# HuiGuanLab/Lite-MKD

Measured on AMD Instinct MI355X. Metric: episodes/sec (5-way 5-shot, 8x224^2 frames), higher is better.
Workload: dtype f32

## Files before the change

### lite-mkd_amd/csrc/norm_pool.hip

```cpp
#include "common.h"
#include <vector>
#include <cmath>
#include <algorithm>

#define NP_THREADS 256
static int g_ew_wg_per_cu = 4;
extern "C" int lmkd_set_elementwise_wg_per_cu(int n) {
  LMKD_REQUIRE(n >= 1 && n <= 8, "lmkd_set_elementwise_wg_per_cu: %d outside 1..8 (the BatchNorm partial buffers hold 2048 rows)", n);
  g_ew_wg_per_cu = n;
  return LMKD_OK;
}
static inline int ew_grid(long n_items) {
  long g = (n_items + NP_THREADS - 1) / NP_THREADS;
  if (g > 256 * g_ew_wg_per_cu) g = 256 * g_ew_wg_per_cu;
  if (g < 1) g = 1;
  return (int)g;
}

extern "C" long lmkd_amax_words(void) { return 2 * LMKD_AMAX_SEG_WORDS; }
static inline unsigned* amd_out(const lmkd_amax_desc* d) { return d ? (unsigned*)d->out_words : nullptr; }
static inline const unsigned* amd_ref(const lmkd_amax_desc* d) { return (d && d->out_words) ? (const unsigned*)d->ref_words : nullptr; }

#define LMKD_FENCE_MAX 128
struct FenceArgs { const unsigned* w[LMKD_FENCE_MAX]; unsigned* r[LMKD_FENCE_MAX]; };
// ... 425 lines not shown
  LMKD_REQUIRE(partial && stats && scratch && tickets && T > 0 && C > 0 && count > 0, "lmkd_bn_finalize: bad arguments");
  LMKD_REQUIRE(cdiv(2 * C, CS_COLS) <= LMKD_TICKET_WORDS, "lmkd_bn_finalize: C=%d exceeds the ticket buffer", C);
  hipLaunchKernelGGL(bn_finalize_kernel, dim3(cdiv(2 * C, CS_COLS), cs_slices(T)), dim3(CS_COLS, CS_LANES), 0, (hipStream_t)stream, partial, T,
                     C, (double)count, gamma, beta, running_mean, running_var, momentum, eps, stats, scratch, tickets, 0, 0.0, 0, 0, bin, bout,
                     bout && amd ? (const unsigned*)amd->ref_words : nullptr);
  LMKD_CHECK_LAUNCH("bn_finalize_kernel");
  return LMKD_OK;
}

extern "C" int lmkd_bn_finalize_seg(const float* partial, int T, int T0, int C, long count0, long count1, const float* gamma, const float* beta,
                                    float eps, float* stats, double* scratch, unsigned* tickets, void* stream, const lmkd_amax_desc* amd) {
  const unsigned* bin = amd ? (const unsigned*)amd->x_words : nullptr;
  unsigned* bout = amd ? (unsigned*)amd->out_words : nullptr;
  if (!bin || !bout) { bin = nullptr; bout = nullptr; }
  LMKD_REQUIRE(partial && stats && scratch && tickets && T0 > 0 && T > T0 && C > 0 && count0 > 0 && count1 > 0, "lmkd_bn_finalize_seg: bad arguments");
  LMKD_REQUIRE(cdiv(2 * C, CS_COLS) <= LMKD_TICKET_WORDS / 2, "lmkd_bn_finalize_seg: C=%d exceeds the ticket buffer", C);
  const int S0 = cs_slices(T0), S1 = cs_slices(T - T0);
  hipLaunchKernelGGL(bn_finalize_kernel, dim3(cdiv(2 * C, CS_COLS), std::max(S0, S1), 2), dim3(CS_COLS, CS_LANES), 0, (hipStream_t)stream, partial, T,
                     C, (double)count0, gamma, beta, (float*)nullptr, (float*)nullptr, 0.f, eps, stats, scratch, tickets, T0, (double)count1, S0, S1, bin, bout,
                     bout && amd ? (const unsigned*)amd->ref_words : nullptr);
  LMKD_CHECK_LAUNCH("bn_finalize_kernel");
  return LMKD_OK;
}

extern "C" int lmkd_bn_eval_stats(int C, const float* gamma, const float* beta, const float* running_mean,
                                  const float* running_var, float eps, float* stats, void* stream) {
  LMKD_REQUIRE(running_mean && running_var && stats && C > 0, "lmkd_bn_eval_stats: bad arguments");
  hipLaunchKernelGGL(bn_eval_stats_kernel, dim3(cdiv(C, 64)), dim3(64), 0, (hipStream_t)stream, C, gamma, beta, running_mean,
                     running_var, eps, stats);
  LMKD_CHECK_LAUNCH("bn_eval_stats_kernel");
  return LMKD_OK;
}

template <typename T>
__global__ void bn_apply_kernel(const T* __restrict__ x, const float* __restrict__ stats, const T* __restrict__ res,
                                const float* __restrict__ rstats, T* __restrict__ y, long n4, int C, int relu, int res_mode,
                                unsigned* __restrict__ mask_bits, long n4_0, unsigned* __restrict__ amax, const unsigned* __restrict__ aref) {
  constexpr int U = ActU<T>::U;
  const int C4 = C >> 2;
  const long nu = n4 / U;
  AmaxStat am = {0.f, 0.f, 0u}, am1 = {0.f, 0.f, 0u};
  const AmaxRef rf0 = amax_ref(aref ? amax_read(aref, 0) : 0u), rf1 = amax_ref(aref ? amax_read(aref, 1) : 0u);
  for (long iu = (long)blockIdx.x * blockDim.x + threadIdx.x; iu < nu; iu += (long)gridDim.x * blockDim.x) {
    float4 v[U], r[U];
    ldv<T, U>(x, iu, v);
    if (res_mode) ldv<T, U>(res, iu, r);
    unsigned nibs = 0;
    const int so = iu * U >= n4_0 ? 5 * C : 0;
#pragma unroll
    for (int u = 0; u < U; ++u) {
      const long i = iu * U + u;
      const int c = (int)(i % C4) * 4 + so;
      const float4 sc = *reinterpret_cast<const float4*>(stats + 2 * C + c);
      const float4 sh = *reinterpret_cast<const float4*>(stats + 3 * C + c);
      float4& w = v[u];
      w.x = fmaf(w.x, sc.x, sh.x); w.y = fmaf(w.y, sc.y, sh.y); w.z = fmaf(w.z, sc.z, sh.z); w.w = fmaf(w.w, sc.w, sh.w);
      if (res_mode == 1) {
        w.x += r[u].x; w.y += r[u].y; w.z += r[u].z; w.w += r[u].w;
      } else if (res_mode == 2) {
        const float4 rs = *reinterpret_cast<const float4*>(rstats + 2 * C + c);
        const float4 rh = *reinterpret_cast<const float4*>(rstats + 3 * C + c);
        w.x += fmaf(r[u].x, rs.x, rh.x); w.y += fmaf(r[u].y, rs.y, rh.y); w.z += fmaf(r[u].z, rs.z, rh.z); w.w += fmaf(r[u].w, rs.w, rh.w);
      }
      if (relu) { w.x = fmaxf(w.x, 0.f); w.y = fmaxf(w.y, 0.f); w.z = fmaxf(w.z, 0.f); w.w = fmaxf(w.w, 0.f); }
      nibs |= ((w.x > 0.f ? 1u : 0u) | (w.y > 0.f ? 2u : 0u) | (w.z > 0.f ? 4u : 0u) | (w.w > 0.f ? 8u : 0u)) << (4 * u);
      if (so) amax_stat4(am1, w, rf1); else amax_stat4(am, w, rf0);
    }
    stv<T, U>(y, iu, v);
    if (mask_bits) {
      constexpr int LPW = 8 / U;
      unsigned wbits = nibs << (4 * U * (threadIdx.x & (LPW - 1)));
      wbits |= __shfl_xor(wbits, 1, 64);
      wbits |= __shfl_xor(wbits, 2, 64);
      if (LPW == 8) wbits |= __shfl_xor(wbits, 4, 64);
      if ((threadIdx.x & (LPW - 1)) == 0) mask_bits[iu / LPW] = wbits;
    }
  }
  if (amax) {
    amax_commit_stat(amax, am, aref != nullptr);
    if (n4_0 < n4) amax_commit_stat(amax + LMKD_AMAX_SEG_WORDS, am1, aref != nullptr);
  }
}

extern "C" int lmkd_bn_apply_seg(const float* x, const float* stats, const float* res, const float* rstats, float* y, long rows, long rows0,
                                 int C, int relu, int res_mode, unsigned* mask_bits, void* stream, const lmkd_amax_desc* amd);
extern "C" int lmkd_bn_apply(const float* x, const float* stats, const float* res, const float* rstats, float* y, long rows,
                             int C, int relu, int res_mode, unsigned* mask_bits, void* stream) {
  return lmkd_bn_apply_seg(x, stats, res, rstats, y, rows, rows, C, relu, res_mode, mask_bits, stream, nullptr);
}
extern "C" int lmkd_bn_apply_seg(const float* x, const float* stats, const float* res, const float* rstats, float* y, long rows, long rows0,
                                 int C, int relu, int res_mode, unsigned* mask_bits, void* stream, const lmkd_amax_desc* amd) {
  unsigned* amax = amd_out(amd);
  const unsigned* aref = amd_ref(amd);
  LMKD_REQUIRE(x && stats && y && rows > 0 && C > 0 && C % 4 == 0, "lmkd_bn_apply: bad arguments (C=%d)", C);
  if (rows0 <= 0 || rows0 > rows) rows0 = rows;
  LMKD_REQUIRE(res_mode == 0 || res, "lmkd_bn_apply: residual pointer missing");
  LMKD_REQUIRE(res_mode != 2 || rstats, "lmkd_bn_apply: residual stats missing");
  LMKD_REQUIRE(!mask_bits || C % 32 == 0, "lmkd_bn_apply: the ReLU bit mask needs C %% 32 == 0 (C=%d)", C);
  LMKD_REQUIRE(!g_lmkd_act_bf16 || C % 8 == 0, "lmkd_bn_apply: bf16 tensors need C %% 8 == 0 (C=%d)", C);
  const long n4 = rows * C / 4;
  if (g_lmkd_act_bf16)
    hipLaunchKernelGGL(bn_apply_kernel<lmkd_bf16_t>, dim3(ew_grid(n4)), dim3(NP_THREADS), 0, (hipStream_t)stream, (const lmkd_bf16_t*)x, stats,
                       (const lmkd_bf16_t*)res, rstats, (lmkd_bf16_t*)y, n4, C, relu, res_mode, mask_bits, rows0 * C / 4, amax, aref);
  else
    hipLaunchKernelGGL(bn_apply_kernel<float>, dim3(ew_grid(n4)), dim3(NP_THREADS), 0, (hipStream_t)stream, x, stats, res, rstats, y, n4, C,
                       relu, res_mode, mask_bits, rows0 * C / 4, amax, aref);
  LMKD_CHECK_LAUNCH("bn_apply_kernel");
  return LMKD_OK;
}

template <typename T>
__device__ __forceinline__ float4 bn_masked_grad(const float4 dy, const float4 xv, const T* yact, long i, const float* stats,
                                                 int C, int c, int mask_mode) {
  float4 g = dy;
  if (mask_mode == 3) {
    const unsigned nib = (reinterpret_cast<const unsigned*>(yact)[i >> 3] >> (4 * (int)(i & 7))) & 15u;
    g.x = (nib & 1u) ? g.x : 0.f; g.y = (nib & 2u) ? g.y : 0.f; g.z = (nib & 4u) ? g.z : 0.f; g.w = (nib & 8u) ? g.w : 0.f;
  } else if (mask_mode == 1) {
    const float4 yv = ld4<T>(yact, i);
    g.x = yv.x > 0.f ? g.x : 0.f; g.y = yv.y > 0.f ? g.y : 0.f; g.z = yv.z > 0.f ? g.z : 0.f; g.w = yv.w > 0.f ? g.w : 0.f;
  } else if (mask_mode == 2) {
    const float4 sc = *reinterpret_cast<const float4*>(stats + 2 * C + c);
    const float4 sh = *reinterpret_cast<const float4*>(stats + 3 * C + c);
    g.x = fmaf(xv.x, sc.x, sh.x) > 0.f ? g.x : 0.f; g.y = fmaf(xv.y, sc.y, sh.y) > 0.f ? g.y : 0.f;
    g.z = fmaf(xv.z, sc.z, sh.z) > 0.f ? g.z : 0.f; g.w = fmaf(xv.w, sc.w, sh.w) > 0.f ? g.w : 0.f;
  }
  return g;
}

struct BnSeg { long rows0; int nb1; };
template <typename T>
__global__ void bn_bwd_reduce_kernel(const T* __restrict__ dy, const T* __restrict__ x, const T* __restrict__ yact,
                                     const float* __restrict__ stats, float* __restrict__ partial, long rows, int C, int CC,
                                     int mask_mode, int nbv, BnSeg sg) {
  extern __shared__ float sm[];
  constexpr int U = ActU<T>::U;
  if (gridDim.z > 1) {
    if (blockIdx.z) {
      const long eo = sg.rows0 * C;
      dy += eo; x += eo;
      if (yact) yact = mask_mode == 3 ? reinterpret_cast<const T*>(reinterpret_cast<const unsigned*>(yact) + eo / 32) : yact + eo;
      stats += 5 * C; partial += (long)2048 * 2 * C; rows -= sg.rows0; nbv = sg.nb1;
    } else {
      rows = sg.rows0;
    }
  }
  const int C4 = C >> 2, CCV = CC / (4 * U);
  const int RL = NP_THREADS / CCV, RL1 = RL / U;
  const int cq = threadIdx.x % CCV, rl = threadIdx.x / CCV;
  const int bv = blockIdx.x * U + rl / RL1, vl = rl % RL1;
  const int c0 = blockIdx.y * CC;
  const int c = c0 + cq * 4 * U;
  float4 s1[U], s2[U], mean[U], istd[U];
#pragma unroll
  for (int u = 0; u < U; ++u) {
    s1[u] = make_float4(0, 0, 0, 0); s2[u] = make_float4(0, 0, 0, 0);
    mean[u] = *reinterpret_cast<const float4*>(stats + c + 4 * u);
    istd[u] = *reinterpret_cast<const float4*>(stats + C + c + 4 * u);
  }
  for (long r = bv < nbv ? (long)bv * RL1 + vl : rows; r < rows; r += (long)nbv * RL1) {
    const long i0 = r * C4 + (c >> 2);
    float4 xv[U], dv[U];
    ldv<T, U>(x, i0 / U, xv);
    ldv<T, U>(dy, i0 / U, dv);
#pragma unroll
    for (int u = 0; u < U; ++u) {
      const float4 g = bn_masked_grad<T>(dv[u], xv[u], yact, i0 + u, stats, C, c + 4 * u, mask_mode);
      s1[u].x += g.x; s1[u].y += g.y; s1[u].z += g.z; s1[u].w += g.w;
      s2[u].x = fmaf(g.x, (xv[u].x - mean[u].x) * istd[u].x, s2[u].x); s2[u].y = fmaf(g.y, (xv[u].y - mean[u].y) * istd[u].y, s2[u].y);
      s2[u].z = fmaf(g.z, (xv[u].z - mean[u].z) * istd[u].z, s2[u].z); s2[u].w = fmaf(g.w, (xv[u].w - mean[u].w) * istd[u].w, s2[u].w);
    }
  }
#pragma unroll
  for (int u = 0; u < U; ++u) {
    float* d = sm + ((long)rl * CC + cq * 4 * U + 4 * u) * 2;
    d[0] = s1[u].x; d[1] = s2[u].x; d[2] = s1[u].y; d[3] = s2[u].y; d[4] = s1[u].z; d[5] = s2[u].z; d[6] = s1[u].w; d[7] = s2[u].w;
  }
  __syncthreads();
  for (int j = threadIdx.x; j < 2 * CC; j += NP_THREADS) {
#pragma unroll
    for (int h = 0; h < U; ++h) {
      if (blockIdx.x * U + h >= nbv) break;
      float s = 0.f;
      for (int q = h * RL1; q < (h + 1) * RL1; ++q) s += sm[(long)q * 2 * CC + j];
      partial[(long)(blockIdx.x * U + h) * 2 * C + 2 * c0 + j] = s;
    }
  }
}

// ... 1 lines not shown
__global__ void bn_bwd_coef_kernel(const float* __restrict__ part, int T, int C, double count, const float* __restrict__ gamma,
                                   const float* __restrict__ stats, float* __restrict__ coef, float* __restrict__ dgamma,
                                   float* __restrict__ dbeta, int accumulate, double* __restrict__ scratch, unsigned* __restrict__ tickets,
                                   CoefSeg cs) {
  __shared__ double sm[CS_LANES][CS_COLS];
  __shared__ double tot[CS_COLS];
  __shared__ int s_last;
  int S = 0;
  const bool seg = gridDim.z > 1;
  if (seg) {
    if (blockIdx.z) { part += cs.pstride; T = cs.T1; count = cs.count1; stats += 5 * C; coef += 5 * C; scratch += (long)(CS_MAX_SLICES + 2) * 2 * C; tickets += LMKD_TICKET_WORDS / 2; S = cs.S1; }
    else S = cs.S0;
  }
  if (!colsum_ticket(part, T, 2 * C, scratch, tickets, sm, tot, &s_last, nullptr, S)) return;
  const int c = blockIdx.x * (CS_COLS / 2) + threadIdx.x;
  if (threadIdx.y != 0 || threadIdx.x >= CS_COLS / 2 || c >= C) return;
  const double sg = tot[2 * threadIdx.x], sgx = tot[2 * threadIdx.x + 1];
  const float g = gamma ? gamma[c] : 1.f;
  const float invstd = stats[C + c];
  coef[c] = g * invstd;
  coef[C + c] = (float)(sg / count);
  coef[2 * C + c] = (float)(sgx / count);
  if (seg) {
    coef[3 * C + c] = (float)sgx;
    coef[4 * C + c] = (float)sg;
    return;
  }
  if (dgamma) dgamma[c] = accumulate ? dgamma[c] + (float)sgx : (float)sgx;
  if (dbeta) dbeta[c] = accumulate ? dbeta[c] + (float)sg : (float)sg;
}

struct ParamGradSeg { float* dgamma; float* dbeta; int accumulate; };
__device__ __forceinline__ void bn_param_grads_seg(const float* __restrict__ coef, int C, const ParamGradSeg& pg) {
  if (blockIdx.x != 0 || !pg.dgamma) return;
  for (int c = threadIdx.x; c < C; c += blockDim.x) {
    const float gx = coef[3 * C + c] + coef[5 * C + 3 * C + c], g = coef[4 * C + c] + coef[5 * C + 4 * C + c];
    pg.dgamma[c] = pg.accumulate ? pg.dgamma[c] + gx : gx;
    if (pg.dbeta) pg.dbeta[c] = pg.accumulate ? pg.dbeta[c] + g : g;
  }
}

template <typename T>
__global__ void bn_bwd_apply_kernel(const T* __restrict__ dy, const T* __restrict__ x, const T* __restrict__ yact,
                                    const float* __restrict__ stats, const float* __restrict__ coef, T* __restrict__ dx,
                                    T* __restrict__ g_out, long n4, int C, int mask_mode, long n4_0, ParamGradSeg pg,
                                    unsigned* __restrict__ amax, const unsigned* __restrict__ aref) {
  constexpr int U = ActU<T>::U;
  const int C4 = C >> 2;
  const long nu = n4 / U;
  if (n4_0 < n4) bn_param_grads_seg(coef, C, pg);
  AmaxStat am = {0.f, 0.f, 0u}, am1 = {0.f, 0.f, 0u};
  const AmaxRef rf0 = amax_ref(aref ? amax_read(aref, 0) : 0u), rf1 = amax_ref(aref ? amax_read(aref, 1) : 0u);
  for (long iu = (long)blockIdx.x * blockDim.x + threadIdx.x; iu < nu; iu += (long)gridDim.x * blockDim.x) {
    float4 xv[U], dv[U], o[U], gq[U];
    ldv<T, U>(x, iu, xv);
    ldv<T, U>(dy, iu, dv);
    const int so = iu * U >= n4_0 ? 5 * C : 0;
    const float* st = stats + so;
    const float* cf = coef + so;
#pragma unroll
    for (int u = 0; u < U; ++u) {
      const long i = iu * U + u;
      const int c = (int)(i % C4) * 4;
      const float4 g = bn_masked_grad<T>(dv[u], xv[u], yact, i, st, C, c, mask_mode);
      const float4 mean = *reinterpret_cast<const float4*>(st + c);
      const float4 istd = *reinterpret_cast<const float4*>(st + C + c);
      const float4 A = *reinterpret_cast<const float4*>(cf + c);
      const float4 mg = *reinterpret_cast<const float4*>(cf + C + c);
      const float4 mgx = *reinterpret_cast<const float4*>(cf + 2 * C + c);
      o[u].x = A.x * (g.x - mg.x - (xv[u].x - mean.x) * istd.x * mgx.x);
      o[u].y = A.y * (g.y - mg.y - (xv[u].y - mean.y) * istd.y * mgx.y);
      o[u].z = A.z * (g.z - mg.z - (xv[u].z - mean.z) * istd.z * mgx.z);
      o[u].w = A.w * (g.w - mg.w - (xv[u].w - mean.w) * istd.w * mgx.w);
      gq[u] = g;
      if (so) amax_stat4(am1, o[u], rf1); else amax_stat4(am, o[u], rf0);
    }
    stv<T, U>(dx, iu, o);
    if (g_out) stv<T, U>(g_out, iu, gq);
  }
  if (amax) {
    amax_commit_stat(amax, am, aref != nullptr);
    if (n4_0 < n4) amax_commit_stat(amax + LMKD_AMAX_SEG_WORDS, am1, aref != nullptr);
  }
}

extern "C" long lmkd_bn_bwd_workspace(int C) { return (long)(2048 * 2 * C) * sizeof(float) + (long)(66 * 2 * C) * sizeof(double) + 64; }

static int bn_bwd_stats_impl(const float* dy, const float* x, const float* yact, const float* stats, const float* gamma, float* dgamma,
                             float* dbeta, float* coef, void* workspace, unsigned* tickets, long rows, long count, int C, int mask_mode,
                             int accumulate_param_grads, hipStream_t s, const char* who, long rows0 = 0, long count0 = 0) {
  LMKD_REQUIRE(dy && x && stats && coef && workspace && tickets, "%s: null pointer", who);
  const bool seg = rows0 > 0 && rows0 < rows;
  LMKD_REQUIRE(!seg || cdiv(2 * C, CS_COLS) <= LMKD_TICKET_WORDS / 2, "%s: C=%d exceeds the ticket buffer", who, C);
  const int CC = C > 1024 ? 1024 : C;
  const int U = g_lmkd_act_bf16 ? 2 : 1;
  LMKD_REQUIRE(C % (4 * U) == 0 && C % CC == 0 && 256 % (CC / 4) == 0, "%s: unsupported channel count %d", who, C);
  LMKD_REQUIRE((mask_mode != 1 && mask_mode != 3) || yact, "%s: mask_mode 1 / 3 needs the activation output / its bit mask", who);
  LMKD_REQUIRE(mask_mode != 3 || C % 32 == 0, "%s: bit masks need C %% 32 == 0", who);
  LMKD_REQUIRE(cdiv(2 * C, CS_COLS) <= LMKD_TICKET_WORDS, "%s: C=%d exceeds the ticket buffer", who, C);
  const int RL1 = NP_THREADS / (CC / 4), RL = RL1 * U;
  auto blocks = [&](long r) {
    int nb = cdiv(r, (long)RL1 * 8);
    if (nb > 256 * g_ew_wg_per_cu * 2) nb = 256 * g_ew_wg_per_cu * 2;
    if (nb > 2048) nb = 2048;
    return nb < 1 ? 1 : nb;
  };
  const int nb = blocks(seg ? rows0 : rows), nb1 = seg ? blocks(rows - rows0) : 0;
  const int nbx = std::max(nb, nb1);
  float* partial = (float*)workspace;
  double* dscr = (double*)((char*)workspace + (((long)(seg ? 2 : 1) * 2048 * 2 * C * sizeof(float) + 63) / 64) * 64);
  BnSeg bs;
  bs.rows0 = seg ? rows0 : rows; bs.nb1 = nb1;
  const int gz = seg ? 2 : 1;
  if (g_lmkd_act_bf16)
    hipLaunchKernelGGL(bn_bwd_reduce_kernel<lmkd_bf16_t>, dim3(cdiv(nbx, 2), C / CC, gz), dim3(NP_THREADS), (size_t)RL * CC * 2 * sizeof(float), s,
                       (const lmkd_bf16_t*)dy, (const lmkd_bf16_t*)x, (const lmkd_bf16_t*)yact, stats, partial, rows, C, CC, mask_mode, nb, bs);
  else
    hipLaunchKernelGGL(bn_bwd_reduce_kernel<float>, dim3(nbx, C / CC, gz), dim3(NP_THREADS), (size_t)RL * CC * 2 * sizeof(float), s, dy, x, yact,
                       stats, partial, rows, C, CC, mask_mode, nb, bs);
  LMKD_CHECK_LAUNCH("bn_bwd_reduce_kernel");
  CoefSeg cs;
  cs.T1 = nb1; cs.pstride = (long)2048 * 2 * C; cs.count1 = (double)(count - count0); cs.S0 = cs_slices(nb); cs.S1 = seg ? cs_slices(nb1) : 0;
  hipLaunchKernelGGL(bn_bwd_coef_kernel, dim3(cdiv(2 * C, CS_COLS), std::max(cs.S0, cs.S1), gz), dim3(CS_COLS, CS_LANES), 0, s, (const float*)partial, nb, C,
                     (double)(seg ? count0 : count), gamma, stats, coef, dgamma, dbeta, accumulate_param_grads, dscr, tickets, cs);
  LMKD_CHECK_LAUNCH("bn_bwd_coef_kernel");
  return LMKD_OK;
}

extern "C" int lmkd_bn_backward_seg(const float* dy, const float* x, const float* yact, const float* stats, const float* gamma, float* dx,
                                    float* g_out, float* dgamma, float* dbeta, float* coef, void* workspace, unsigned* tickets, long rows,
                                    long rows0, int C, int mask_mode, int accumulate_param_grads, void* stream, const lmkd_amax_desc* amd);
extern "C" int lmkd_bn_backward(const float* dy, const float* x, const float* yact, const float* stats, const float* gamma,
                                float* dx, float* g_out, float* dgamma, float* dbeta, float* coef, void* workspace, unsigned* tickets,
                                long rows, int C, int mask_mode, int accumulate_param_grads, void* stream) {
  return lmkd_bn_backward_seg(dy, x, yact, stats, gamma, dx, g_out, dgamma, dbeta, coef, workspace, tickets, rows, rows, C, mask_mode,
                              accumulate_param_grads, stream, nullptr);
}
extern "C" int lmkd_bn_backward_seg(const float* dy, const float* x, const float* yact, const float* stats, const float* gamma, float* dx,
                                    float* g_out, float* dgamma, float* dbeta, float* coef, void* workspace, unsigned* tickets, long rows,
                                    long rows0, int C, int mask_mode, int accumulate_param_grads, void* stream, const lmkd_amax_desc* amd) {
  unsigned* amax = amd_out(amd);
  const unsigned* aref = amd_ref(amd);
  LMKD_REQUIRE(dx, "lmkd_bn_backward: null pointer");
  hipStream_t s = (hipStream_t)stream;
  if (rows0 <= 0 || rows0 >= rows) rows0 = rows;
  const int rc = bn_bwd_stats_impl(dy, x, yact, stats, gamma, dgamma, dbeta, coef, workspace, tickets, rows, rows, C, mask_mode,
                                   accumulate_param_grads, s, "lmkd_bn_backward", rows0, rows0);
  if (rc) return rc;
  const long n4 = rows * C / 4, n4_0 = rows0 * C / 4;
  ParamGradSeg pg;
  pg.dgamma = dgamma; pg.dbeta = dbeta; pg.accumulate = accumulate_param_grads;
  if (g_lmkd_act_bf16)
    hipLaunchKernelGGL(bn_bwd_apply_kernel<lmkd_bf16_t>, dim3(ew_grid(n4)), dim3(NP_THREADS), 0, s, (const lmkd_bf16_t*)dy, (const lmkd_bf16_t*)x,
                       (const lmkd_bf16_t*)yact, stats, (const float*)coef, (lmkd_bf16_t*)dx, (lmkd_bf16_t*)g_out, n4, C, mask_mode, n4_0, pg, amax, aref);
  else
    hipLaunchKernelGGL(bn_bwd_apply_kernel<float>, dim3(ew_grid(n4)), dim3(NP_THREADS), 0, s, dy, x, yact, stats, (const float*)coef, dx, g_out,
                       n4, C, mask_mode, n4_0, pg, amax, aref);
  LMKD_CHECK_LAUNCH("bn_bwd_apply_kernel");
  return LMKD_OK;
}

extern "C" int lmkd_bn_backward_part_seg(const float* part, int T, int T0, const float* dy, const float* x, const float* stats, const float* gamma,
                                         float* dx, float* dgamma, float* dbeta, float* coef, void* workspace, unsigned* tickets, long rows,
                                         long rows0, int C, int accumulate_param_grads, void* stream, const lmkd_amax_desc* amd);
extern "C" int lmkd_bn_backward_part(const float* part, int T, const float* dy, const float* x, const float* stats, const float* gamma,
                                     float* dx, float* dgamma, float* dbeta, float* coef, void* workspace, unsigned* tickets, long rows, int C,
                                     int accumulate_param_grads, void* stream) {
  return lmkd_bn_backward_part_seg(part, T, T, dy, x, stats, gamma, dx, dgamma, dbeta, coef, workspace, tickets, rows, rows, C,
                                   accumulate_param_grads, stream, nullptr);
}
extern "C" int lmkd_bn_backward_part_seg(const float* part, int T, int T0, const float* dy, const float* x, const float* stats, const float* gamma,
                                         float* dx, float* dgamma, float* dbeta, float* coef, void* workspace, unsigned* tickets, long rows,
                                         long rows0, int C, int accumulate_param_grads, void* stream, const lmkd_amax_desc* amd) {
  unsigned* amax = amd_out(amd);
  const unsigned* aref = amd_ref(amd);
  LMKD_REQUIRE(part && T > 0 && dy && x && stats && dx && coef && workspace && tickets, "lmkd_bn_backward_part: null pointer");
  LMKD_REQUIRE(!g_lmkd_act_bf16 && C % 4 == 0, "lmkd_bn_backward_part: fp32 tensors, C %% 4 == 0");
  const bool seg = T0 > 0 && T0 < T && rows0 > 0 && rows0 < rows;
  LMKD_REQUIRE(seg || (T0 == T && rows0 == rows), "lmkd_bn_backward_part_seg: T0 / rows0 must both name a split or both the whole");
  LMKD_REQUIRE(cdiv(2 * C, CS_COLS) <= LMKD_TICKET_WORDS / (seg ? 2 : 1), "lmkd_bn_backward_part: C=%d exceeds the ticket buffer", C);
  hipStream_t s = (hipStream_t)stream;
  double* dscr = (double*)((char*)workspace + (((long)2048 * 2 * C * sizeof(float) + 63) / 64) * 64);
  CoefSeg cs;
  cs.T1 = T - T0; cs.pstride = (long)T0 * 2 * C; cs.count1 = (double)(rows - rows0); cs.S0 = cs_slices(T0); cs.S1 = seg ? cs_slices(T - T0) : 0;
  hipLaunchKernelGGL(bn_bwd_coef_kernel, dim3(cdiv(2 * C, CS_COLS), std::max(cs.S0, cs.S1), seg ? 2 : 1), dim3(CS_COLS, CS_LANES), 0, s, part, T0, C,
                     (double)rows0, gamma, stats, coef, dgamma, dbeta, accumulate_param_grads, dscr, tickets, cs);
  LMKD_CHECK_LAUNCH("bn_bwd_coef_kernel");
  const long n4 = rows * C / 4;
  ParamGradSeg pg;
  pg.dgamma = dgamma; pg.dbeta = dbeta; pg.accumulate = accumulate_param_grads;
  hipLaunchKernelGGL(bn_bwd_apply_kernel<float>, dim3(ew_grid(n4)), dim3(NP_THREADS), 0, s, dy, x, (const float*)nullptr, stats, (const float*)coef,
                     dx, (float*)nullptr, n4, C, 2, rows0 * C / 4, pg, amax, aref);
  LMKD_CHECK_LAUNCH("bn_bwd_apply_kernel");
  return LMKD_OK;
}

extern "C" int lmkd_bn_backward_stats(const float* dy, const float* cmax, const float* stats, const float* gamma, float* dgamma, float* dbeta,
                                      float* coef, void* workspace, unsigned* tickets, long pooled_rows, long count, int C,
                                      int accumulate_param_grads, void* stream) {
  LMKD_REQUIRE(pooled_rows > 0 && count >= pooled_rows, "lmkd_bn_backward_stats: bad row counts");
  return bn_bwd_stats_impl(dy, cmax, nullptr, stats, gamma, dgamma, dbeta, coef, workspace, tickets, pooled_rows, count, C, 2,
                           accumulate_param_grads, (hipStream_t)stream, "lmkd_bn_backward_stats");
}
extern "C" int lmkd_bn_backward_stats_seg(const float* dy, const float* cmax, const float* stats, const float* gamma, float* coef, void* workspace,
                                          unsigned* tickets, long pooled_rows, long pooled_rows0, long count, long count0, int C, void* stream) {
  LMKD_REQUIRE(pooled_rows0 > 0 && pooled_rows0 < pooled_rows && count0 >= pooled_rows0 && count - count0 >= pooled_rows - pooled_rows0,
               "lmkd_bn_backward_stats_seg: bad row counts");
  return bn_bwd_stats_impl(dy, cmax, nullptr, stats, gamma, nullptr, nullptr, coef, workspace, tickets, pooled_rows, count, C, 2, 0,
                           (hipStream_t)stream, "lmkd_bn_backward_stats_seg", pooled_rows0, count0);
}

template <typename T>
__global__ void relu_bwd_kernel(const T* __restrict__ dy, const T* __restrict__ y, T* __restrict__ g, long n4) {
  for (long i = (long)blockIdx.x * blockDim.x + threadIdx.x; i < n4; i += (long)gridDim.x * blockDim.x) {
    const float4 d = ld4<T>(dy, i), v = ld4<T>(y, i);
    st4<T>(g, i, make_float4(v.x > 0.f ? d.x : 0.f, v.y > 0.f ? d.y : 0.f, v.z > 0.f ? d.z : 0.f, v.w > 0.f ? d.w : 0.f));
  }
}
extern "C" int lmkd_relu_backward(const float* dy, const float* y, float* g, long n, void* stream) {
  LMKD_REQUIRE(dy && y && g && n > 0 && n % 4 == 0, "lmkd_relu_backward: bad arguments");
  if (g_lmkd_act_bf16)
    hipLaunchKernelGGL(relu_bwd_kernel<lmkd_bf16_t>, dim3(ew_grid(n / 4)), dim3(NP_THREADS), 0, (hipStream_t)stream, (const lmkd_bf16_t*)dy,
                       (const lmkd_bf16_t*)y, (lmkd_bf16_t*)g, n / 4);
  else
    hipLaunchKernelGGL(relu_bwd_kernel<float>, dim3(ew_grid(n / 4)), dim3(NP_THREADS), 0, (hipStream_t)stream, dy, y, g, n / 4);
  LMKD_CHECK_LAUNCH("relu_bwd_kernel");
  return LMKD_OK;
}

template <typename T>
__global__ void bn_relu_maxpool_kernel(const T* __restrict__ x, const float* __restrict__ stats, T* __restrict__ y,
                                       uchar4* __restrict__ idx, T* __restrict__ cmax, int N, int H, int W, int C, int OH, int OW, int N0,
                                       unsigned* __restrict__ amax, const unsigned* __restrict__ aref) {
  constexpr int U = ActU<T>::U;
  const int CU = C / (4 * U);
  const long total = (long)N * OH * OW * CU;
  AmaxStat amx = {0.f, 0.f, 0u}, amx1 = {0.f, 0.f, 0u};
  const AmaxRef rf0 = amax_ref(aref ? amax_read(aref, 0) : 0u), rf1 = amax_ref(aref ? amax_read(aref, 1) : 0u);
  for (long i = (long)blockIdx.x * blockDim.x + threadIdx.x; i < total; i += (long)gridDim.x * blockDim.x) {
    const int cq = (int)(i % CU);
    long r = i / CU;
    const int ow = (int)(r % OW); r /= OW;
    const int oh = (int)(r % OH);
    const int n = (int)(r / OH);
    float4 sc[U], sh[U], m[U], cm[U];
    uchar4 am[U];
#pragma unroll
    for (int u = 0; u < U; ++u) {
      const float* st = stats + (n >= N0 ? 5 * C : 0);
      sc[u] = *reinterpret_cast<const float4*>(st + 2 * C + (cq * U + u) * 4);
      sh[u] = *reinterpret_cast<const float4*>(st + 3 * C + (cq * U + u) * 4);
      m[u] = make_float4(-INFINITY, -INFINITY, -INFINITY, -INFINITY);
      cm[u] = make_float4(0.f, 0.f, 0.f, 0.f);
      am[u] = make_uchar4(255, 255, 255, 255);
    }
#pragma unroll
    for (int kh = 0; kh < 3; ++kh) {
      const int h = oh * 2 - 1 + kh;
      if ((unsigned)h >= (unsigned)H) continue;
#pragma unroll
      for (int kw = 0; kw < 3; ++kw) {
        const int w = ow * 2 - 1 + kw;
        if ((unsigned)w >= (unsigned)W) continue;
        float4 rr[U];
        ldv<T, U>(x, ((long)(n * H + h) * W + w) * CU + cq, rr);
        const unsigned char t = (unsigned char)(kh * 3 + kw);
#pragma unroll
        for (int u = 0; u < U; ++u) {
          const float4 r4 = rr[u];
          float4 v;
          v.x = fmaxf(fmaf(r4.x, sc[u].x, sh[u].x), 0.f); v.y = fmaxf(fmaf(r4.y, sc[u].y, sh[u].y), 0.f);
          v.z = fmaxf(fmaf(r4.z, sc[u].z, sh[u].z), 0.f); v.w = fmaxf(fmaf(r4.w, sc[u].w, sh[u].w), 0.f);
          if (v.x > m[u].x || am[u].x == 255) { m[u].x = v.x; am[u].x = t; cm[u].x = r4.x; }
          if (v.y > m[u].y || am[u].y == 255) { m[u].y = v.y; am[u].y = t; cm[u].y = r4.y; }
          if (v.z > m[u].z || am[u].z == 255) { m[u].z = v.z; am[u].z = t; cm[u].z = r4.z; }
          if (v.w > m[u].w || am[u].w == 255) { m[u].w = v.w; am[u].w = t; cm[u].w = r4.w; }
        }
      }
    }
    stv<T, U>(y, i, m);
#pragma unroll
    for (int u = 0; u < U; ++u) {
      idx[i * U + u] = am[u];
      if (n >= N0) amax_stat4(amx1, m[u], rf1); else amax_stat4(amx, m[u], rf0);
    }
    if (cmax) stv<T, U>(cmax, i, cm);
  }
  if (amax) {
    amax_commit_stat(amax, amx, aref != nullptr);
    if (N0 < N) amax_commit_stat(amax + LMKD_AMAX_SEG_WORDS, amx1, aref != nullptr);
  }
}

extern "C" int lmkd_bn_relu_maxpool_fwd_seg(const float* x, const float* stats, float* y, unsigned char* idx, float* cmax, int N, int N0, int H,
                                            int W, int C, void* stream, const lmkd_amax_desc* amd);
extern "C" int lmkd_bn_relu_maxpool_fwd(const float* x, const float* stats, float* y, unsigned char* idx, float* cmax, int N, int H, int W,
                                        int C, void* stream) {
  return lmkd_bn_relu_maxpool_fwd_seg(x, stats, y, idx, cmax, N, N, H, W, C, stream, nullptr);
}
extern "C" int lmkd_bn_relu_maxpool_fwd_seg(const float* x, const float* stats, float* y, unsigned char* idx, float* cmax, int N, int N0, int H,
                                            int W, int C, void* stream, const lmkd_amax_desc* amd) {
  unsigned* amax = amd_out(amd);
  const unsigned* aref = amd_ref(amd);
  LMKD_REQUIRE(x && stats && y && idx && C % (g_lmkd_act_bf16 ? 8 : 4) == 0, "lmkd_bn_relu_maxpool_fwd: bad arguments");
  if (N0 <= 0 || N0 > N) N0 = N;
  const int OH = (H + 2 - 3) / 2 + 1, OW = (W + 2 - 3) / 2 + 1;
  const long total = (long)N * OH * OW * C / (g_lmkd_act_bf16 ? 8 : 4);
  if (g_lmkd_act_bf16)
    hipLaunchKernelGGL(bn_relu_maxpool_kernel<lmkd_bf16_t>, dim3(ew_grid(total)), dim3(NP_THREADS), 0, (hipStream_t)stream, (const lmkd_bf16_t*)x,
                       stats, (lmkd_bf16_t*)y, (uchar4*)idx, (lmkd_bf16_t*)cmax, N, H, W, C, OH, OW, N0, amax, aref);
  else
    hipLaunchKernelGGL(bn_relu_maxpool_kernel<float>, dim3(ew_grid(total)), dim3(NP_THREADS), 0, (hipStream_t)stream, x, stats, y, (uchar4*)idx,
                       cmax, N, H, W, C, OH, OW, N0, amax, aref);
  LMKD_CHECK_LAUNCH("bn_relu_maxpool_kernel");
  return LMKD_OK;
}

template <typename T>
__global__ void maxpool_bwd_kernel(const T* __restrict__ dy, const uchar4* __restrict__ idx, T* __restrict__ g, int N, int H,
                                   int W, int C, int OH, int OW) {
  const int C4 = C >> 2;
  const long total = (long)N * H * W * C4;
  for (long i = (long)blockIdx.x * blockDim.x + threadIdx.x; i < total; i += (long)gridDim.x * blockDim.x) {
    const int cq = (int)(i % C4);
    long r = i / C4;
    const int w = (int)(r % W); r /= W;
    const int h = (int)(r % H);
    const int n = (int)(r / H);
    float4 acc = make_float4(0.f, 0.f, 0.f, 0.f);
    const int oh_lo = h >> 1, oh_hi = (h + 1) >> 1;
    const int ow_lo = w >> 1, ow_hi = (w + 1) >> 1;
    for (int oh = oh_lo; oh <= oh_hi; ++oh) {
      if (oh >= OH) continue;
      const int kh = h - (2 * oh - 1);
      for (int ow = ow_lo; ow <= ow_hi; ++ow) {
        if (ow >= OW) continue;
        const int kw = w - (2 * ow - 1);
        const unsigned char t = (unsigned char)(kh * 3 + kw);
        const long o = ((long)(n * OH + oh) * OW + ow) * C4 + cq;
        const uchar4 am = idx[o];
        const float4 d = ld4<T>(dy, o);
        if (am.x == t) acc.x += d.x;
        if (am.y == t) acc.y += d.y;
        if (am.z == t) acc.z += d.z;
        if (am.w == t) acc.w += d.w;
      }
    }
    st4<T>(g, i, acc);
  }
}

template <typename T>
__global__ void stem_unpool_bn_bwd_kernel(const T* __restrict__ dy, const uchar4* __restrict__ idx, const T* __restrict__ c,
                                          const float* __restrict__ stats, const float* __restrict__ coef, T* __restrict__ dc, int N,
                                          int H, int W, int C, int OH, int OW, int N0, ParamGradSeg pg, unsigned* __restrict__ amax,
                                          const unsigned* __restrict__ aref) {
  const int C4 = C >> 2;
  const int HB = (H + 1) >> 1, WB = (W + 1) >> 1;
  const long total = (long)N * HB * WB * C4;
  AmaxStat amx = {0.f, 0.f, 0u}, amx1 = {0.f, 0.f, 0u};
  const AmaxRef rf0 = amax_ref(aref ? amax_read(aref, 0) : 0u), rf1 = amax_ref(aref ? amax_read(aref, 1) : 0u);
  if (N0 < N) bn_param_grads_seg(coef, C, pg);
  for (long i = (long)blockIdx.x * blockDim.x + threadIdx.x; i < total; i += (long)gridDim.x * blockDim.x) {
    const int cq = (int)(i % C4);
    long r = i / C4;
    const int b = (int)(r % WB); r /= WB;
    const int a = (int)(r % HB);
    const int n = (int)(r / HB);
    const int ch = cq * 4 + (n >= N0 ? 5 * C : 0);
    const float4 sc = *reinterpret_cast<const float4*>(stats + 2 * C + ch);
    const float4 sh = *reinterpret_cast<const float4*>(stats + 3 * C + ch);
    const float4 mean = *reinterpret_cast<const float4*>(stats + ch);
    const float4 istd = *reinterpret_cast<const float4*>(stats + C + ch);
    const float4 A = *reinterpret_cast<const float4*>(coef + ch);
    const float4 mg = *reinterpret_cast<const float4*>(coef + C + ch);
    const float4 mgx = *reinterpret_cast<const float4*>(coef + 2 * C + ch);
    float4 d[2][2];
    uchar4 am[2][2];
#pragma unroll
    for (int wi = 0; wi < 2; ++wi)
#pragma unroll
      for (int wj = 0; wj < 2; ++wj) {
        const int oh = a + wi, ow = b + wj;
        if (oh < OH && ow < OW) {
          const long o = ((long)(n * OH + oh) * OW + ow) * C4 + cq;
          d[wi][wj] = ld4<T>(dy, o);
          am[wi][wj] = idx[o];
        } else {
          d[wi][wj] = make_float4(0.f, 0.f, 0.f, 0.f);
          am[wi][wj] = make_uchar4(254, 254, 254, 254);
        }
      }
#pragma unroll
    for (int pi = 0; pi < 2; ++pi) {
      const int h = 2 * a + pi;
      if (h >= H) continue;
// ... 186 lines not shown
```

Before: 51.01.

## Add specialized fp32 BatchNorm apply, backward-apply and BN-ReLU-maxpool kernels with LDS tables

Adds fp32-only kernels for BN apply, BN backward apply and fused BN+ReLU+maxpool. Each block processes one contiguous chunk, keeps the channel index with an incremental counter instead of a modulo, and uses 32-bit byte offsets. Per-channel scale/shift/coef values are staged in shared memory when C<=512. The aim is to cut integer division, 64-bit address arithmetic and redundant global loads of per-channel parameters in these bandwidth-bound passes, at the cost of extra code paths and 32-bit size limits.

```diff
diff --git a/lite-mkd_amd/csrc/norm_pool.hip b/lite-mkd_amd/csrc/norm_pool.hip
--- a/lite-mkd_amd/csrc/norm_pool.hip
+++ b/lite-mkd_amd/csrc/norm_pool.hip
@@ -531,6 +531,96 @@
   }
 }
 
+#define NP_TAB_MAX_C 512
+struct EwChunk { unsigned chunk, cmod; };
+static inline int ew_chunks(long n4, int C4, EwChunk* ck) {
+  const long g = ew_grid(n4);
+  const long chunk = ((n4 + g - 1) / g + NP_THREADS - 1) / NP_THREADS * NP_THREADS;
+  ck->chunk = (unsigned)chunk; ck->cmod = (unsigned)(chunk % C4);
+  return (int)((n4 + chunk - 1) / chunk);
+}
+#define LMKD_REQUIRE_EW32(n4, who) LMKD_REQUIRE((n4) < (1L << 31), "%s: %ld groups of 4 elements exceed the 32-bit offsets of the fp32 pass", who, (long)(n4))
+template <bool L>
+__device__ __forceinline__ float4 ew_row(const float4* __restrict__ s, const float* __restrict__ g, int row, int C4, unsigned c4) {
+  if constexpr (L) return s[row * C4 + c4];
+  else return reinterpret_cast<const float4*>(g)[row * C4 + c4];
+}
+__device__ __forceinline__ void ew_stage(float4* __restrict__ s, const float* __restrict__ g, int n) {
+  for (int j = threadIdx.x; j < n; j += NP_THREADS) s[j] = reinterpret_cast<const float4*>(g)[j];
+}
+__device__ __forceinline__ float4 ew_ld(const float4* __restrict__ b, unsigned ob) {
+  asm volatile("" : "+v"(ob));
+  return *reinterpret_cast<const float4*>(reinterpret_cast<const char*>(b) + ob);
+}
+__device__ __forceinline__ void ew_st(float4* __restrict__ b, unsigned ob, const float4& v) {
+  asm volatile("" : "+v"(ob));
+  *reinterpret_cast<float4*>(reinterpret_cast<char*>(b) + ob) = v;
+}
+__device__ __forceinline__ bool ew_range(int seg, long b0, long b1, long split, long& lo, long& hi) {
+  lo = seg ? (b0 > split ? b0 : split) : b0;
+  hi = seg ? b1 : (b1 < split ? b1 : split);
+  return lo < hi;
+}
+
+template <bool L>
+__global__ void __launch_bounds__(NP_THREADS) bn_apply_f32_kernel(const float4* __restrict__ x, const float* __restrict__ stats,
+                                                                  const float4* __restrict__ res, const float* __restrict__ rstats,
+                                                                  float4* __restrict__ y, long n4, int C4, int relu, int res_mode,
+                                                                  unsigned* __restrict__ mask_bits, long n4_0, EwChunk ck,
+                                                                  unsigned* __restrict__ amax, const unsigned* __restrict__ aref) {
+  extern __shared__ float4 ew_tab[];
+  const long b0 = (long)blockIdx.x * ck.chunk;
+  const long b1 = b0 + ck.chunk < n4 ? b0 + ck.chunk : n4;
+  const unsigned step = NP_THREADS % C4;
+  for (int seg = 0; seg < 2; ++seg) {
+    long lo, hi;
+    if (!ew_range(seg, b0, b1, n4_0, lo, hi)) continue;
+    const float* st = stats + (seg ? 20 * C4 : 0) + 8 * C4;
+    const float* rt = rstats ? rstats + (seg ? 20 * C4 : 0) + 8 * C4 : nullptr;
+    if (L) {
+      if (seg) __syncthreads();
+      ew_stage(ew_tab, st, 2 * C4);
+      if (res_mode == 2) ew_stage(ew_tab + 2 * C4, rt, 2 * C4);
+      __syncthreads();
+    }
+    const AmaxRef rf = amax_ref(aref ? amax_read(aref, seg) : 0u);
+    AmaxStat am = {0.f, 0.f, 0u};
+    const float4* xb = x + lo;
+    const float4* rb = res + lo;
+    float4* yb = y + lo;
+    unsigned* mb = mask_bits + (lo >> 3);
+    const unsigned n = (unsigned)(hi - lo);
+    unsigned c4 = ((lo == b0 ? blockIdx.x * ck.cmod : 0u) + threadIdx.x) % C4;
+    for (unsigned ob = threadIdx.x * 16u; ob < n * 16u; ob += NP_THREADS * 16u) {
+      float4 w = ew_ld(xb, ob);
+      {
+        const float4 sc = ew_row<L>(ew_tab, st, 0, C4, c4), sh = ew_row<L>(ew_tab, st, 1, C4, c4);
+        w.x = fmaf(w.x, sc.x, sh.x); w.y = fmaf(w.y, sc.y, sh.y); w.z = fmaf(w.z, sc.z, sh.z); w.w = fmaf(w.w, sc.w, sh.w);
+      }
+      if (res_mode == 1) {
+        const float4 r = ew_ld(rb, ob);
+        w.x += r.x; w.y += r.y; w.z += r.z; w.w += r.w;
+      } else if (res_mode == 2) {
+        const float4 r = ew_ld(rb, ob);
+        const float4 rs = ew_row<L>(ew_tab + 2 * C4, rt, 0, C4, c4), rh = ew_row<L>(ew_tab + 2 * C4, rt, 1, C4, c4);
+        w.x += fmaf(r.x, rs.x, rh.x); w.y += fmaf(r.y, rs.y, rh.y); w.z += fmaf(r.z, rs.z, rh.z); w.w += fmaf(r.w, rs.w, rh.w);
+      }
+      if (relu) { w.x = fmaxf(w.x, 0.f); w.y = fmaxf(w.y, 0.f); w.z = fmaxf(w.z, 0.f); w.w = fmaxf(w.w, 0.f); }
+      ew_st(yb, ob, w);
+      if (mask_bits) {
+        unsigned wbits = ((w.x > 0.f ? 1u : 0u) | (w.y > 0.f ? 2u : 0u) | (w.z > 0.f ? 4u : 0u) | (w.w > 0.f ? 8u : 0u)) << (4 * (threadIdx.x & 7));
+        wbits |= __shfl_xor(wbits, 1, 64);
+        wbits |= __shfl_xor(wbits, 2, 64);
+        wbits |= __shfl_xor(wbits, 4, 64);
+        if ((threadIdx.x & 7) == 0) mb[ob >> 7] = wbits;
+      }
+      amax_stat4(am, w, rf);
+      c4 += step; if (c4 >= (unsigned)C4) c4 -= C4;
+    }
+    if (amax) amax_commit_stat(amax + seg * LMKD_AMAX_SEG_WORDS, am, aref != nullptr);
+  }
+}
+
 extern "C" int lmkd_bn_apply_seg(const float* x, const float* stats, const float* res, const float* rstats, float* y, long rows, long rows0,
                                  int C, int relu, int res_mode, unsigned* mask_bits, void* stream, const lmkd_amax_desc* amd);
 extern "C" int lmkd_bn_apply(const float* x, const float* stats, const float* res, const float* rstats, float* y, long rows,
@@ -551,9 +641,17 @@
   if (g_lmkd_act_bf16)
     hipLaunchKernelGGL(bn_apply_kernel<lmkd_bf16_t>, dim3(ew_grid(n4)), dim3(NP_THREADS), 0, (hipStream_t)stream, (const lmkd_bf16_t*)x, stats,
                        (const lmkd_bf16_t*)res, rstats, (lmkd_bf16_t*)y, n4, C, relu, res_mode, mask_bits, rows0 * C / 4, amax, aref);
-  else
-    hipLaunchKernelGGL(bn_apply_kernel<float>, dim3(ew_grid(n4)), dim3(NP_THREADS), 0, (hipStream_t)stream, x, stats, res, rstats, y, n4, C,
-                       relu, res_mode, mask_bits, rows0 * C / 4, amax, aref);
+  else {
+    LMKD_REQUIRE_EW32(n4, "lmkd_bn_apply");
+    EwChunk ck;
+    const int C4 = C / 4, g = ew_chunks(n4, C4, &ck);
+    if (C <= NP_TAB_MAX_C)
+      hipLaunchKernelGGL(bn_apply_f32_kernel<true>, dim3(g), dim3(NP_THREADS), (size_t)(res_mode == 2 ? 4 : 2) * C4 * sizeof(float4), (hipStream_t)stream,
+                         (const float4*)x, stats, (const float4*)res, rstats, (float4*)y, n4, C4, relu, res_mode, mask_bits, rows0 * C4, ck, amax, aref);
+    else
+      hipLaunchKernelGGL(bn_apply_f32_kernel<false>, dim3(g), dim3(NP_THREADS), 0, (hipStream_t)stream, (const float4*)x, stats, (const float4*)res,
+                         rstats, (float4*)y, n4, C4, relu, res_mode, mask_bits, rows0 * C4, ck, amax, aref);
+  }
   LMKD_CHECK_LAUNCH("bn_apply_kernel");
   return LMKD_OK;
 }
@@ -721,6 +819,91 @@
     amax_commit_stat(amax, am, aref != nullptr);
     if (n4_0 < n4) amax_commit_stat(amax + LMKD_AMAX_SEG_WORDS, am1, aref != nullptr);
   }
+}
+
+template <bool L>
+__device__ __forceinline__ float4 bwd_row(const float4* __restrict__ s, const float* __restrict__ g, int row, int C4, unsigned c4) {
+  if constexpr (L) return s[c4 * 7 + row];
+  else return reinterpret_cast<const float4*>(g)[(row & 3) * C4 + c4];
+}
+template <bool L>
+__global__ void __launch_bounds__(NP_THREADS) bn_bwd_apply_f32_kernel(const float4* __restrict__ dy, const float4* __restrict__ x,
+                                                                      const float* __restrict__ yact, const float* __restrict__ stats,
+                                                                      const float* __restrict__ coef, float4* __restrict__ dx,
+                                                                      float4* __restrict__ g_out, long n4, int C4, int mask_mode, long n4_0,
+                                                                      EwChunk ck, ParamGradSeg pg, unsigned* __restrict__ amax,
+                                                                      const unsigned* __restrict__ aref) {
+  extern __shared__ float4 ew_tab[];
+  if (n4_0 < n4) bn_param_grads_seg(coef, 4 * C4, pg);
+  const long b0 = (long)blockIdx.x * ck.chunk;
+  const long b1 = b0 + ck.chunk < n4 ? b0 + ck.chunk : n4;
+  const unsigned step = NP_THREADS % C4;
+  for (int seg = 0; seg < 2; ++seg) {
+    long lo, hi;
+    if (!ew_range(seg, b0, b1, n4_0, lo, hi)) continue;
+    const float* st = stats + (seg ? 20 * C4 : 0);
+    const float* cf = coef + (seg ? 20 * C4 : 0);
+    if (L) {
+      if (seg) __syncthreads();
+      for (int j = threadIdx.x; j < 7 * C4; j += NP_THREADS) {
+        const int row = j / C4, cg = j - row * C4;
+        ew_tab[cg * 7 + row] = row < 4 ? reinterpret_cast<const float4*>(st)[j] : reinterpret_cast<const float4*>(cf)[j - 4 * C4];
+      }
+      __syncthreads();
+    }
+    const AmaxRef rf = amax_ref(aref ? amax_read(aref, seg) : 0u);
+    AmaxStat am = {0.f, 0.f, 0u};
+    const float4* xb = x + lo;
+    const float4* db = dy + lo;
+    const float4* yb = reinterpret_cast<const float4*>(yact) + lo;
+    const unsigned* mb = reinterpret_cast<const unsigned*>(yact) + (lo >> 3);
+    float4* dxb = dx + lo;
+    float4* gb = g_out + lo;
+    const unsigned n = (unsigned)(hi - lo);
+    unsigned c4 = ((lo == b0 ? blockIdx.x * ck.cmod : 0u) + threadIdx.x) % C4;
+    for (unsigned ob = threadIdx.x * 16u; ob < n * 16u; ob += NP_THREADS * 16u) {
+      const float4 xv = ew_ld(xb, ob);
+      float4 g = ew_ld(db, ob);
+      if (mask_mode == 3) {
+        const unsigned nib = (mb[ob >> 7] >> ((ob >> 2) & 28u)) & 15u;
+        g.x = (nib & 1u) ? g.x : 0.f; g.y = (nib & 2u) ? g.y : 0.f; g.z = (nib & 4u) ? g.z : 0.f; g.w = (nib & 8u) ? g.w : 0.f;
+      } else if (mask_mode == 1) {
+        const float4 yv = ew_ld(yb, ob);
+        g.x = yv.x > 0.f ? g.x : 0.f; g.y = yv.y > 0.f ? g.y : 0.f; g.z = yv.z > 0.f ? g.z : 0.f; g.w = yv.w > 0.f ? g.w : 0.f;
+      } else if (mask_mode == 2) {
+        const float4 sc = bwd_row<L>(ew_tab, st, 2, C4, c4), sh = bwd_row<L>(ew_tab, st, 3, C4, c4);
+        g.x = fmaf(xv.x, sc.x, sh.x) > 0.f ? g.x : 0.f; g.y = fmaf(xv.y, sc.y, sh.y) > 0.f ? g.y : 0.f;
+        g.z = fmaf(xv.z, sc.z, sh.z) > 0.f ? g.z : 0.f; g.w = fmaf(xv.w, sc.w, sh.w) > 0.f ? g.w : 0.f;
+      }
+      if (g_out) ew_st(gb, ob, g);
+      float4 t;
+      { const float4 r = bwd_row<L>(ew_tab, st, 0, C4, c4); t.x = xv.x - r.x; t.y = xv.y - r.y; t.z = xv.z - r.z; t.w = xv.w - r.w; }
+      { const float4 r = bwd_row<L>(ew_tab, st, 1, C4, c4); t.x *= r.x; t.y *= r.y; t.z *= r.z; t.w *= r.w; }
+      { const float4 r = bwd_row<L>(ew_tab, cf, 6, C4, c4); t.x *= r.x; t.y *= r.y; t.z *= r.z; t.w *= r.w; }
+      { const float4 r = bwd_row<L>(ew_tab, cf, 5, C4, c4); g.x -= r.x; g.y -= r.y; g.z -= r.z; g.w -= r.w; }
+      g.x -= t.x; g.y -= t.y; g.z -= t.z; g.w -= t.w;
+      { const float4 r = bwd_row<L>(ew_tab, cf, 4, C4, c4); g.x = r.x * g.x; g.y = r.y * g.y; g.z = r.z * g.z; g.w = r.w * g.w; }
+      ew_st(dxb, ob, g);
+      amax_stat4(am, g, rf);
+      c4 += step; if (c4 >= (unsigned)C4) c4 -= C4;
+    }
+    if (amax) amax_commit_stat(amax + seg * LMKD_AMAX_SEG_WORDS, am, aref != nullptr);
+  }
+}
+
+static int bn_bwd_apply_f32(const float* dy, const float* x, const float* yact, const float* stats, const float* coef, float* dx, float* g_out,
+                            long n4, int C, int mask_mode, long n4_0, const ParamGradSeg& pg, unsigned* amax, const unsigned* aref, hipStream_t s) {
+  LMKD_REQUIRE_EW32(n4, "lmkd_bn_backward");
+  EwChunk ck;
+  const int C4 = C / 4, g = ew_chunks(n4, C4, &ck);
+  if (C <= NP_TAB_MAX_C)
+    hipLaunchKernelGGL(bn_bwd_apply_f32_kernel<true>, dim3(g), dim3(NP_THREADS), (size_t)7 * C4 * sizeof(float4), s, (const float4*)dy, (const float4*)x, yact,
+                       stats, coef, (float4*)dx, (float4*)g_out, n4, C4, mask_mode, n4_0, ck, pg, amax, aref);
+  else
+    hipLaunchKernelGGL(bn_bwd_apply_f32_kernel<false>, dim3(g), dim3(NP_THREADS), 0, s, (const float4*)dy, (const float4*)x, yact, stats, coef, (float4*)dx,
+                       (float4*)g_out, n4, C4, mask_mode, n4_0, ck, pg, amax, aref);
+  LMKD_CHECK_LAUNCH("bn_bwd_apply_kernel");
+  return LMKD_OK;
 }
 
 extern "C" long lmkd_bn_bwd_workspace(int C) { return (long)(2048 * 2 * C) * sizeof(float) + (long)(66 * 2 * C) * sizeof(double) + 64; }
@@ -793,8 +976,7 @@
     hipLaunchKernelGGL(bn_bwd_apply_kernel<lmkd_bf16_t>, dim3(ew_grid(n4)), dim3(NP_THREADS), 0, s, (const lmkd_bf16_t*)dy, (const lmkd_bf16_t*)x,
                        (const lmkd_bf16_t*)yact, stats, (const float*)coef, (lmkd_bf16_t*)dx, (lmkd_bf16_t*)g_out, n4, C, mask_mode, n4_0, pg, amax, aref);
   else
-    hipLaunchKernelGGL(bn_bwd_apply_kernel<float>, dim3(ew_grid(n4)), dim3(NP_THREADS), 0, s, dy, x, yact, stats, (const float*)coef, dx, g_out,
-                       n4, C, mask_mode, n4_0, pg, amax, aref);
+    return bn_bwd_apply_f32(dy, x, yact, stats, coef, dx, g_out, n4, C, mask_mode, n4_0, pg, amax, aref, s);
   LMKD_CHECK_LAUNCH("bn_bwd_apply_kernel");
   return LMKD_OK;
 }
@@ -828,10 +1010,7 @@
   const long n4 = rows * C / 4;
   ParamGradSeg pg;
   pg.dgamma = dgamma; pg.dbeta = dbeta; pg.accumulate = accumulate_param_grads;
-  hipLaunchKernelGGL(bn_bwd_apply_kernel<float>, dim3(ew_grid(n4)), dim3(NP_THREADS), 0, s, dy, x, (const float*)nullptr, stats, (const float*)coef,
-                     dx, (float*)nullptr, n4, C, 2, rows0 * C / 4, pg, amax, aref);
-  LMKD_CHECK_LAUNCH("bn_bwd_apply_kernel");
-  return LMKD_OK;
+  return bn_bwd_apply_f32(dy, x, nullptr, stats, coef, dx, nullptr, n4, C, 2, rows0 * C / 4, pg, amax, aref, s);
 }
 
 extern "C" int lmkd_bn_backward_stats(const float* dy, const float* cmax, const float* stats, const float* gamma, float* dgamma, float* dbeta,
@@ -931,6 +1110,77 @@
   }
 }
 
+struct PoolDiv { FastDiv c4, ow, oh; };
+template <bool L>
+__global__ void __launch_bounds__(NP_THREADS) bn_relu_maxpool_f32_kernel(const float4* __restrict__ x, const float* __restrict__ stats,
+                                                                         float4* __restrict__ y, uchar4* __restrict__ idx,
+                                                                         float4* __restrict__ cmax, unsigned total, unsigned split, int H, int W,
+                                                                         int C4, int OH, int OW, PoolDiv dv, EwChunk ck,
+                                                                         unsigned* __restrict__ amax, const unsigned* __restrict__ aref) {
+  extern __shared__ float4 ew_tab[];
+  const unsigned b0 = blockIdx.x * ck.chunk;
+  const unsigned b1 = b0 + ck.chunk < total ? b0 + ck.chunk : total;
+  for (int seg = 0; seg < 2; ++seg) {
+    const unsigned lo = seg ? (b0 > split ? b0 : split) : b0, hi = seg ? b1 : (b1 < split ? b1 : split);
+    if (lo >= hi) continue;
+    const float* st = stats + (seg ? 20 * C4 : 0) + 8 * C4;
+    if (L) {
+      if (seg) __syncthreads();
+      for (int j = threadIdx.x; j < 2 * C4; j += NP_THREADS) ew_tab[j < C4 ? 2 * j : 2 * (j - C4) + 1] = reinterpret_cast<const float4*>(st)[j];
+      __syncthreads();
+    }
+    const AmaxRef rf = amax_ref(aref ? amax_read(aref, seg) : 0u);
+    AmaxStat ams = {0.f, 0.f, 0u};
+    const unsigned nf = lo / (unsigned)(OH * OW * C4);
+    const float4* xb = x + (long)nf * H * W * C4;
+    float4* yb = y + lo;
+    float4* cb = cmax + lo;
+    uchar4* ib = idx + lo;
+    const unsigned n = hi - lo;
+    for (unsigned o = threadIdx.x; o < n; o += NP_THREADS) {
+      unsigned r = fdiv(lo + o, dv.c4);
+      const unsigned cq = lo + o - r * C4;
+      unsigned q = fdiv(r, dv.ow);
+      const int ow = (int)(r - q * OW);
+      r = fdiv(q, dv.oh);
+      const int oh = (int)(q - r * OH);
+      const unsigned fr = (r - nf) * H;
+      float4 sc, sh;
+      if constexpr (L) { sc = ew_tab[2 * cq]; sh = ew_tab[2 * cq + 1]; }
+      else { sc = reinterpret_cast<const float4*>(st)[cq]; sh = reinterpret_cast<const float4*>(st)[C4 + cq]; }
+      float4 m = make_float4(-INFINITY, -INFINITY, -INFINITY, -INFINITY);
+      float4 cm = make_float4(0.f, 0.f, 0.f, 0.f);
+      unsigned am = 0xFFFFFFFFu;
+#pragma unroll 1
+      for (int kh = 0; kh < 3; ++kh) {
+        const int h = oh * 2 - 1 + kh;
+        if ((unsigned)h >= (unsigned)H) continue;
+#pragma unroll 1
+        for (int kw = 0; kw < 3; ++kw) {
+          const int w = ow * 2 - 1 + kw;
+          if ((unsigned)w >= (unsigned)W) continue;
+          const float4 r4 = ew_ld(xb, (((fr + h) * W + w) * C4 + cq) * 16u);
+          const unsigned t = (unsigned)(kh * 3 + kw);
+          float v;
+          v = fmaxf(fmaf(r4.x, sc.x, sh.x), 0.f); if (v > m.x || (am & 0xFFu) == 0xFFu) { m.x = v; am = (am & 0xFFFFFF00u) | t; cm.x = r4.x; }
+          v = fmaxf(fmaf(r4.y, sc.y, sh.y), 0.f); if (v > m.y || (am & 0xFF00u) == 0xFF00u) { m.y = v; am = (am & 0xFFFF00FFu) | (t << 8); cm.y = r4.y; }
+          v = fmaxf(fmaf(r4.z, sc.z, sh.z), 0.f); if (v > m.z || (am & 0xFF0000u) == 0xFF0000u) { m.z = v; am = (am & 0xFF00FFFFu) | (t << 16); cm.z = r4.z; }
+          v = fmaxf(fmaf(r4.w, sc.w, sh.w), 0.f); if (v > m.w || (am >> 24) == 0xFFu) { m.w = v; am = (am & 0x00FFFFFFu) | (t << 24); cm.w = r4.w; }
+        }
+      }
+      ew_st(yb, o * 16u, m);
+      {
+        unsigned ob = o * 4u;
+        asm volatile("" : "+v"(ob));
+        *reinterpret_cast<unsigned*>(reinterpret_cast<char*>(ib) + ob) = am;
+      }
+      if (cmax) ew_st(cb, o * 16u, cm);
+      amax_stat4(ams, m, rf);
+    }
+    if (amax) amax_commit_stat(amax + seg * LMKD_AMAX_SEG_WORDS, ams, aref != nullptr);
+  }
+}
+
 extern "C" int lmkd_bn_relu_maxpool_fwd_seg(const float* x, const float* stats, float* y, unsigned char* idx, float* cmax, int N, int N0, int H,
                                             int W, int C, void* stream, const lmkd_amax_desc* amd);
 extern "C" int lmkd_bn_relu_maxpool_fwd(const float* x, const float* stats, float* y, unsigned char* idx, float* cmax, int N, int H, int W,
@@ -948,9 +1198,22 @@
   if (g_lmkd_act_bf16)
     hipLaunchKernelGGL(bn_relu_maxpool_kernel<lmkd_bf16_t>, dim3(ew_grid(total)), dim3(NP_THREADS), 0, (hipStream_t)stream, (const lmkd_bf16_t*)x,
                        stats, (lmkd_bf16_t*)y, (uchar4*)idx, (lmkd_bf16_t*)cmax, N, H, W, C, OH, OW, N0, amax, aref);
-  else
-    hipLaunchKernelGGL(bn_relu_maxpool_kernel<float>, dim3(ew_grid(total)), dim3(NP_THREADS), 0, (hipStream_t)stream, x, stats, y, (uchar4*)idx,
-                       cmax, N, H, W, C, OH, OW, N0, amax, aref);
+  else {
+    const int C4 = C / 4;
+    LMKD_REQUIRE_EW32(total, "lmkd_bn_relu_maxpool_fwd");
+    LMKD_REQUIRE((long)H * W * C4 < (1L << 27), "lmkd_bn_relu_maxpool_fwd: a frame of %d x %d x %d exceeds the 32-bit offsets of the fp32 pass", H, W, C);
+    EwChunk ck;
+    const int g = ew_chunks(total, C4, &ck);
+    PoolDiv dv;
+    dv.c4 = make_fastdiv(C4); dv.ow = make_fastdiv(OW); dv.oh = make_fastdiv(OH);
+    const unsigned split = (unsigned)((long)N0 * OH * OW * C4);
+    if (C <= NP_TAB_MAX_C)
+      hipLaunchKernelGGL(bn_relu_maxpool_f32_kernel<true>, dim3(g), dim3(NP_THREADS), (size_t)2 * C4 * sizeof(float4), (hipStream_t)stream, (const float4*)x,
+                         stats, (float4*)y, (uchar4*)idx, (float4*)cmax, (unsigned)total, split, H, W, C4, OH, OW, dv, ck, amax, aref);
+    else
+      hipLaunchKernelGGL(bn_relu_maxpool_f32_kernel<false>, dim3(g), dim3(NP_THREADS), 0, (hipStream_t)stream, (const float4*)x, stats, (float4*)y,
+                         (uchar4*)idx, (float4*)cmax, (unsigned)total, split, H, W, C4, OH, OW, dv, ck, amax, aref);
+  }
   LMKD_CHECK_LAUNCH("bn_relu_maxpool_kernel");
   return LMKD_OK;
 }
```

Result: no change. 51.51 (median of 6 runs) (+1.0%).
